# dRaniwal/RAJNI-ViT

Measured on AMD Instinct MI355X. Metric: images/sec ViT-B/16@224 with README schedule, higher is better.
Workload: dtype bf16

## Files before the change

include/rajni_hip_debug.h:

```cpp
#ifndef RAJNI_HIP_DEBUG_H
#define RAJNI_HIP_DEBUG_H

#include "rajni_hip.h"

#ifdef __cplusplus
extern "C" {
#endif

void rajni_debug_force_attention(int mode);

int rajni_debug_attention_rows(const void* qkv, const int32_t* keep_idx, void* out, int B, int n_src, int np, int nq,
                               int H, int D, float scale, int dtype, rajni_stream_t stream);

void rajni_debug_set_last_block_all_rows(int on);
int rajni_debug_last_block_cls_rows(const rajni_vit_plan* plan, const rajni_vit_ext* ext, const rajni_vit_prefix* prefix);

void rajni_debug_force_gemm_tiling(int mode);

void rajni_debug_force_f8_tiling(int mode);

void rajni_debug_set_resid_stagger(int units);

void rajni_debug_set_gemm_nblock_bytes(int bytes);

enum { RAJNI_TILING_SMALL = 1,
       RAJNI_TILING_F32 = 2,
       RAJNI_TILING_WIDE = 4,
       RAJNI_TILING_MID = 5,
       RAJNI_TILING_F8_STREAM = 8,
       RAJNI_TILING_F8_WIDE = 9 };
typedef struct rajni_linear_plan {
  int tiling;
  int tiles_n, total_tiles, nblk;
  int grid;
  int lds_bytes;
} rajni_linear_plan;
int rajni_debug_linear_plan(const rajni_linear_args* args, int cus, rajni_linear_plan* out);

void rajni_debug_force_score_two_pass(int on);

void rajni_debug_force_score_tiled(int on);

void rajni_debug_set_gemm_stamps(void* buf);

#ifdef __cplusplus
}
#endif
#endif
```

rajni-vit_amd/csrc/common.h:

```cpp
#pragma once
#include <hip/hip_runtime.h>
#include <stdint.h>
#include <stdio.h>
#include "../../include/rajni_hip.h"
#include "../../include/rajni_hip_debug.h"

typedef unsigned short bf16_t;
typedef __attribute__((ext_vector_type(8))) __bf16 bf16x8;
typedef __attribute__((ext_vector_type(2))) __bf16 bf16x2;
typedef __attribute__((ext_vector_type(4))) float f32x4;
typedef __attribute__((ext_vector_type(16))) float f32x16;
typedef __attribute__((ext_vector_type(4))) short s16x4;

#define LDS_PTR(p) ((__attribute__((address_space(3))) void*)(p))
#define GLB_PTR(p) ((const __attribute__((address_space(1))) void*)(p))

__device__ __forceinline__ float bf2f(bf16_t u) { return __uint_as_float(((unsigned)u) << 16); }
__device__ __forceinline__ bf16_t f2bf(float f) {
  __bf16 b = (__bf16)f;
  return __builtin_bit_cast(bf16_t, b);
}
__device__ __forceinline__ unsigned pack2bf(float lo, float hi) {
  bf16x2 v = {(__bf16)lo, (__bf16)hi};
  return __builtin_bit_cast(unsigned, v);
// ... 116 lines not shown
  KC_GEMM_BIAS = 0, KC_GEMM_GELU = 1, KC_GEMM_RESID = 2, KC_GEMM_PATCH = 3, KC_ATTENTION = 4,
  KC_LAYERNORM = 5, KC_SCORE_SELECT = 6, KC_IMPORTANCE = 7, KC_SELECT = 8, KC_GATHER = 9,
  KC_CLS_POS = 10, KC_OTHER = 11,
  KC_GEMM_RESID_SQ = 12,
  KC_GEMM8_BIAS = 13, KC_GEMM8_GELU = 14, KC_GEMM8_RESID = 15,
  KC_GEMM8_RESID_SQ = 16
};
struct ProfScope {
  int kc; hipStream_t s; void* rec;
  ProfScope(int kclass, hipStream_t stream, double flops, double bytes);
  ~ProfScope();
};

#define RAJNI_CHECK_LAUNCH(name)                                              \
  do {                                                                        \
    hipError_t e__ = hipGetLastError();                                       \
    if (e__ != hipSuccess) {                                                  \
      rajni_set_error("%s launch failed: %s", name, hipGetErrorString(e__));  \
      return RAJNI_ERR_LAUNCH;                                                \
    }                                                                         \
  } while (0)

#define RAJNI_REQUIRE(cond, code, ...)       \
  do {                                       \
    if (!(cond)) {                           \
      rajni_set_error(__VA_ARGS__);          \
      return code;                           \
    }                                        \
  } while (0)

extern unsigned long long* rajni_g_stamps;

int launch_linear(const rajni_linear_args& a, hipStream_t s);
int launch_patch_embed(const void* images, const void* w, const float* bias, const void* cls,
                       const void* pos, int pos_has_cls, void* x, int out_f32, int B, int Cin, int S,
                       int P, int C, int dtype, void* ws, size_t ws_bytes, hipStream_t s,
                       int num_prefix = 1, const void* reg = nullptr);
size_t patch_embed_workspace_bytes(int B, int Cin, int S, int P, int dtype);
int launch_layernorm(const void* x, long xs, const float* w, const float* b, void* y, int rows,
                     int C, float eps, int x_f32, int dtype, hipStream_t s);
int launch_layernorm_fp8(const void* x, long xs, const float* w, const float* b, void* yq, float* yscale,
                         float* hscale, float wnorm, float bmax, int rows, int C, float eps, int x_f32, hipStream_t s);
int launch_attention(const void* qkv, const int32_t* keep_idx, void* out, int B, int n_src, int np, int nq,
                     int H, int D, float scale, int dtype, hipStream_t s);
int launch_attention_fp8(const void* qkv, const int32_t* keep_idx, void* out_q, float out_scale, float* row_scale,
                         int B, int n_src, int np, int H, int D, float scale, hipStream_t s);
int launch_attention_cls(const void* qkv, void* out, int B, int N, int H, int D, float scale, int dtype,
                         hipStream_t s, float q_scale = 0.f);
int launch_score_select(const void* qkv, const void* scores_in, int B, int N, int H, int D,
                        float eps, int keep, void* scores_out, int32_t* keep_idx,
                        void* next_scores, int dtype, hipStream_t s, int num_prefix = 1, void* ws = nullptr,
                        size_t ws_bytes = 0);
int launch_gather_rows(const void* src, const int32_t* idx, void* dst, int B, int n_src, int n_dst,
                       int row_bytes, hipStream_t s);
int launch_qk_norm(void* qkv, const float* qw, const float* qb, const float* kw, const float* kb, int rows, int H, int D,
                   float eps, int dtype, hipStream_t s);
int launch_layernorm_stream(void* x, const float* w, const float* b, int rows, int C, float eps, int x_f32, int dtype, hipStream_t s);
int launch_pool_norm(const void* x, int B, int N, int C, int pool, const float* nw, const float* nb, float neps,
                     const float* fw, const float* fb, float feps, void* out, int x_f32, int dtype, hipStream_t s,
                     int num_prefix = 1);
```

rajni-vit_amd/csrc/forward.hip:

```cpp
#include "common.h"

namespace {

inline size_t align256(size_t v) { return (v + 255) & ~(size_t)255; }

struct Workspace {
  char *xa, *xb, *xn, *qkv, *att, *hid, *clsn, *scf, *cols;
  char* sst; size_t sst_bytes;
  float *xs, *hs;
  size_t total, cols_bytes;
};

Workspace carve(const rajni_vit_plan& p, int P) {
  const size_t gw = p.img_size / p.patch_size, n0 = gw * gw + P;
  const size_t rows = (size_t)p.B * n0, es = p.dtype == RAJNI_F32 ? 4 : 2, xs = (p.dtype == RAJNI_F32 || !p.resid_bf16) ? 4 : 2;
  Workspace w{};
  size_t off = 0;
  auto take = [&](size_t bytes) { size_t o = off; off += align256(bytes); return o; };
  const size_t oxa = take(rows * p.C * xs), oxb = take(rows * p.C * xs), oxn = take(rows * p.C * es);
  const size_t oqkv = take(rows * 3 * p.C * es), oatt = take(rows * p.C * es);
  const size_t ohid = take(rows * p.hidden * es), ocls = take((size_t)p.B * p.C * es);
  const size_t oscf = take(rows * es);
  w.cols_bytes = patch_embed_workspace_bytes(p.B, p.in_chans, p.img_size, p.patch_size, p.dtype);
  const size_t ocols = take(w.cols_bytes);
// ... 99 lines not shown
}
rajni_linear_args fc1_args(const Fwd& f, const rajni_block& blk, int M) {
  rajni_linear_args g = linear_args(f.p.dtype, f.w.xn, blk.fc1_w, blk.fc1_b, blk.fc1_s, f.w.hid, M, f.p.hidden, f.p.C, RAJNI_EPI_BIAS_GELU);
  if (f.p.act_fp8) { g.x_scale = f.w.xs; g.y_scale = f.w.hs; }
  return g;
}
rajni_linear_args fc2_args(const Fwd& f, const rajni_block& blk, int M, void* y) {
  rajni_linear_args g = linear_args(f.p.dtype, f.w.hid, blk.fc2_w, blk.fc2_b, blk.fc2_s, y, M, f.p.C, f.p.hidden, RAJNI_EPI_BIAS_RESID);
  if (f.p.act_fp8) g.x_scale = f.w.hs;
  g.gamma = blk.ls2; g.resid = y; g.ldr = f.p.C; g.stream_f32 = f.sf32;
  return g;
}

int layernorm(const Fwd& f, const void* x, const float* g, const float* b, int rows, float* hs = nullptr, float wnorm = 0.f,
              float bmax = 0.f) {
  const rajni_vit_plan& p = f.p;
  if (p.act_fp8) return launch_layernorm_fp8(x, p.C, g, b, f.w.xn, f.w.xs, hs, wnorm, bmax, rows, p.C, p.ln_eps, f.sf32, f.s);
  return launch_layernorm(x, p.C, g, b, f.w.xn, rows, p.C, p.ln_eps, f.sf32, p.dtype, f.s);
}

inline bool attn_emits_e4m3(const rajni_vit_plan& p, const rajni_block& blk, int np) {
  return p.act_fp8 && blk.attn_out_scale > 0.f && blk.proj_s != nullptr && p.D == 64 && np <= 224;
}

struct Tail { rajni_linear_args proj, fc1, fc2; };
Tail tail_args(const Fwd& f, const rajni_block& blk, const AttnRows& r, const void* x, void* y) {
  return Tail{proj_args(f, blk, r, x, y), fc1_args(f, blk, r.M), fc2_args(f, blk, r.M, y)};
}
bool tail_ok(const Tail& t) {
  rajni_linear_plan unused;
  return rajni_debug_linear_plan(&t.proj, 256, &unused) == RAJNI_OK && rajni_debug_linear_plan(&t.fc1, 256, &unused) == RAJNI_OK &&
         rajni_debug_linear_plan(&t.fc2, 256, &unused) == RAJNI_OK;
}
int launch_tail(const Fwd& f, const rajni_block& blk, const Tail& t) {
  int rc = launch_linear(t.proj, f.s);
  if (rc != RAJNI_OK) return rc;
  rc = layernorm(f, t.proj.y, blk.norm2_w, blk.norm2_b, t.proj.M, f.w.hs, blk.fc1_rownorm_max, blk.fc1_bias_absmax);
  if (rc != RAJNI_OK) return rc;
  rc = launch_linear(t.fc1, f.s);
  if (rc != RAJNI_OK) return rc;
  return launch_linear(t.fc2, f.s);
}

inline int prefix_count(const rajni_vit_prefix* pre) { return (pre && pre->num_prefix > 1) ? pre->num_prefix : 1; }

int check_prefix(const rajni_vit_prefix* pre, const char* who) {
  if (!pre) return RAJNI_OK;
  RAJNI_REQUIRE(pre->num_prefix >= 0 && pre->num_prefix <= RAJNI_MAX_PREFIX, RAJNI_ERR_INVALID,
                "%s: num_prefix must be 0..%d (%d)", who, RAJNI_MAX_PREFIX, pre->num_prefix);
  RAJNI_REQUIRE(pre->num_prefix <= 1 || pre->reg_token != nullptr, RAJNI_ERR_INVALID,
                "%s: %d prefix tokens but reg_token is null", who, pre->num_prefix);
  RAJNI_REQUIRE(pre->num_prefix > 1 || pre->reg_token == nullptr, RAJNI_ERR_INVALID,
                "%s: reg_token given but num_prefix is %d", who, pre->num_prefix);
  return RAJNI_OK;
}

inline int tokens_after(const rajni_block& blk, int N, int P) { return blk.keep > 0 ? blk.keep + P : N; }
int tokens_entering(const rajni_vit_plan& p, int P, int i) {
  const int gw = p.img_size / p.patch_size;
  int N = gw * gw + P;
  for (int j = 0; j < i; ++j) N = tokens_after(p.blocks[j], N, P);
  return N;
}

inline int logits_stride(const rajni_vit_plan& p) { return p.logits_ld > 0 ? p.logits_ld : p.num_classes; }

int check_schedule(const rajni_vit_plan& p, int P) {
  for (int i = 0; i < p.depth; ++i) {
    const rajni_block& blk = p.blocks[i];
    if (blk.keep <= 0) continue;
    const int patches = tokens_entering(p, P, i) - P;
    RAJNI_REQUIRE(blk.keep <= patches, RAJNI_ERR_INVALID, "block %d: keep=%d but only %d patch tokens", i, blk.keep, patches);
    RAJNI_REQUIRE(blk.keep_idx && blk.next_scores, RAJNI_ERR_INVALID, "block %d: keep_idx/next_scores buffers missing", i);
  }
// ... 66 lines not shown
  const Fwd f{p, w, (dt != RAJNI_F32 && !p.resid_bf16) ? 1 : 0, s};
  int N = tokens_entering(p, P, 0);

  rc = launch_patch_embed(images, p.patch_w, p.patch_b, p.cls_token, p.pos_embed, p.pos_has_cls,
                          w.xa, f.sf32, B, p.in_chans, p.img_size, p.patch_size, C, dt, w.cols, w.cols_bytes, s,
                          P, P > 1 ? pre->reg_token : nullptr);
  if (rc != RAJNI_OK) return rc;
  if (ext && ext->norm_pre_w) {
    rc = launch_layernorm_stream(w.xa, ext->norm_pre_w, ext->norm_pre_b, B * N, C, ext->norm_pre_eps, f.sf32, dt, s);
    if (rc != RAJNI_OK) return rc;
  }

  char* cur = w.xa;
  char* oth = w.xb;
  const void* carried = nullptr;

  for (int i = 0; i < p.depth; ++i) {
    const rajni_block& blk = p.blocks[i];
    if (p.token_counts) p.token_counts[i] = N;
    const int M = B * N;
    rc = layernorm(f, cur, blk.norm1_w, blk.norm1_b, M);
    if (rc != RAJNI_OK) return rc;
    rc = launch_linear(qkv_args(f, blk, M), s);
    if (rc != RAJNI_OK) return rc;
    if (qkn) {
      rc = launch_qk_norm(w.qkv, qkn[i].q_norm_w, qkn[i].q_norm_b, qkn[i].k_norm_w, qkn[i].k_norm_b, M, p.H, p.D, ext->qk_eps, dt, s);
      if (rc != RAJNI_OK) return rc;
    }

    const long cls_ld = (long)N * C;
    if (p.cls_only_last_block && i == p.depth - 1 && blk.keep == 0 && N > 1) {
      rc = launch_attention_cls(w.qkv, w.att, B, N, p.H, p.D, p.attn_scale, dt, s, attn_emits_e4m3(p, blk, N) ? blk.attn_out_scale : 0.f);
      if (rc != RAJNI_OK) return rc;
      rc = launch_tail(f, blk, tail_args(f, blk, AttnRows{B, C, nullptr, cls_ld, nullptr, 0, 0}, cur, oth));
      if (rc != RAJNI_OK) return rc;
      cur = oth; N = 1;
      break;
    }
    if (last_block_cls_rows(p, ext, i, N)) {
      const Tail t = tail_args(f, blk, AttnRows{B, cls_ld, nullptr, cls_ld, nullptr, 0, 0}, cur, oth);
      if (tail_ok(t)) {
        rc = launch_attention(w.qkv, nullptr, w.att, B, N, N, 1, p.H, p.D, p.attn_scale, dt, s);
        if (rc != RAJNI_OK) return rc;
        rc = launch_tail(f, blk, t);
        if (rc != RAJNI_OK) return rc;
        cur = oth; N = 1;
        break;
      }
    }

    const int Np = tokens_after(blk, N, P);
    const int32_t* idx = nullptr;
    if (blk.keep > 0) {
      const bool recompute = blk.update || carried == nullptr;
      if (blk.forced_keep_idx) {
        const void* full = carried;
        if (recompute) {
          void* dst = blk.scores ? blk.scores : (void*)w.scf;
          rc = launch_score_select(w.qkv, nullptr, B, N, p.H, p.D, 1e-6f, 0, dst, nullptr, nullptr, dt, s, 1, w.sst, w.sst_bytes);
          if (rc != RAJNI_OK) return rc;
          full = dst;
        }
        const int n = B * Np;
        if (dt == RAJNI_F32)
          hipLaunchKernelGGL(carry_scores_kernel<float>, dim3((n + 255) / 256), dim3(256), 0, s,
                             (const float*)full, blk.forced_keep_idx, (float*)blk.next_scores, B, N, Np);
        else
          hipLaunchKernelGGL(carry_scores_kernel<bf16_t>, dim3((n + 255) / 256), dim3(256), 0, s,
                             (const bf16_t*)full, blk.forced_keep_idx, (bf16_t*)blk.next_scores, B, N, Np);
        RAJNI_CHECK_LAUNCH("carry_scores_kernel");
        idx = blk.forced_keep_idx;
      } else {
        if (recompute)
          rc = launch_score_select(w.qkv, nullptr, B, N, p.H, p.D, 1e-6f, blk.keep, blk.scores,
                                   blk.keep_idx, blk.next_scores, dt, s, P, w.sst, w.sst_bytes);
        else
          rc = launch_score_select(nullptr, carried, B, N, 0, 0, 0.f, blk.keep, nullptr,
                                   blk.keep_idx, blk.next_scores, dt, s, P);
        if (rc != RAJNI_OK) return rc;
        idx = blk.keep_idx;
      }
      carried = blk.next_scores;
    } else {
      carried = nullptr;
    }

    const bool att8 = attn_emits_e4m3(p, blk, Np);
    if (att8) rc = launch_attention_fp8(w.qkv, idx, w.att, blk.attn_out_scale, w.xs, B, N, Np, p.H, p.D, p.attn_scale, s);
    else rc = launch_attention(w.qkv, idx, w.att, B, N, Np, Np, p.H, p.D, p.attn_scale, dt, s);
    if (rc != RAJNI_OK) return rc;
    char* y = idx ? oth : cur;
    rc = launch_tail(f, blk, tail_args(f, blk, AttnRows{B * Np, C, att8 ? w.xs : nullptr, C, idx, Np, N}, cur, y));
    if (rc != RAJNI_OK) return rc;
    if (idx) { oth = cur; cur = y; }
    N = Np;
  }

  if (ext && (ext->pool != RAJNI_POOL_TOKEN || ext->fc_norm_w || ext->norm_absent))
    rc = launch_pool_norm(cur, B, N, C, ext->pool, ext->norm_absent ? nullptr : p.norm_w, p.norm_b, p.ln_eps,
                          ext->fc_norm_w, ext->fc_norm_b, ext->fc_norm_eps, w.clsn, f.sf32, dt, s, P);
  else
    rc = launch_layernorm(cur, (long)N * C, p.norm_w, p.norm_b, w.clsn, B, C, p.ln_eps, f.sf32, dt, s);
  if (rc != RAJNI_OK) return rc;
  rajni_linear_args head = linear_args(dt, w.clsn, p.head_w, p.head_b, nullptr, logits, B, p.num_classes, C, RAJNI_EPI_BIAS);
  head.ldc = logits_stride(p);
  return launch_linear(head, s);
}

}
```

rajni-vit_amd/csrc/gemm.hip:

```cpp
#include <stdlib.h>
#include <type_traits>
#include "common.h"

namespace {

enum { EPI_BIAS = 0, EPI_GELU = 1, EPI_RESID = 2, EPI_PATCH = 3,
       EPI_GELU8 = 4 };
enum { ALOAD_PLAIN = 0, ALOAD_PATCH = 1 };

struct GemmParams {
  const void* X; long lda;
  const void* W; long ldw;
  const float* wscale;
  const float* xscale;
  const float* yscale;
  const float* bias;
  const float* gamma;
  const void* R; long ldr;
  const int* ridx; int r_np, r_nsrc;
  void* Y; long ldc;
  int M, N, K;
  int tiles_n, total_tiles;
  int nblk;
  int cin, S, log2ps, gw, npatch;
// ... 903 lines not shown
  pre.valid = false;
  stage(0, 0);
  for (int kt = 0; kt < nk; ++kt) {
    asm volatile("s_waitcnt vmcnt(0)" ::: "memory");
    __syncthreads();
    if (kt + 1 < nk) stage(kt + 1, (kt + 1) & 1);
    else prefetch_resid<EPI, SF32, 4>(p, pre, m0 + wm * 64, n0 + wn * 64, l15, g);
    const char* sx = smem + (kt & 1) * STAGE_BYTES;
    const char* sw = sx + TILE_BYTES;
#pragma unroll
    for (int ks = 0; ks < 2; ++ks) {
      const int c = ks * 4 + g;
      bf16x8 xf[4], wf[4];
#pragma unroll
      for (int i = 0; i < 4; ++i) {
        xf[i] = *reinterpret_cast<const bf16x8*>(sx + xoff[i] + ((c ^ xkey[i]) << 4));
        if constexpr (W8)
          wf[i] = w_frag_bf16(*reinterpret_cast<const WFrag*>(sw + woff[i] + (((c >> 1) ^ wkey[i]) << 4) + ((c & 1) << 3)));
        else
          wf[i] = *reinterpret_cast<const bf16x8*>(sw + woff[i] + ((c ^ wkey[i]) << 4));
      }
#pragma unroll
      for (int ni = 0; ni < 4; ++ni)
#pragma unroll
        for (int mi = 0; mi < 4; ++mi)
          acc[ni][mi] = mfma_16x16x32<A>(wf[ni], xf[mi], acc[ni][mi]);
    }
  }

  epilogue_tile<A, EPI, SF32, 4, W8>(p, acc, m0 + wm * 64, n0 + wn * 64, l15, g, pre);
}
}

#include "gemm_f8.h"

namespace f32 {
constexpr int BM = 128, BN = 128, BK = 32;
constexpr int TILE_BYTES = BM * BK * 4;
constexpr int STAGE_BYTES = 2 * TILE_BYTES;
constexpr int LDS_BYTES = 2 * STAGE_BYTES;
using small::key_w;
using small::key_x;

template <int EPI>
__device__ __forceinline__ void epilogue_row_f32(const GemmParams& p, int m, int nb, float* v, const float* gam) {
  long orow = m;
  if (EPI == EPI_GELU) {
#pragma unroll
    for (int j = 0; j < 16; ++j) v[j] = 0.5f * v[j] * (1.0f + erff(v[j] * 0.70710678118654752f));
  } else if (EPI == EPI_RESID) {
    long rrow = m;
    if (p.ridx != nullptr) {
      const int b = m / p.r_np;
      rrow = (long)b * p.r_nsrc + p.ridx[m];
    }
    const long roff = rrow * p.ldr + nb;
#pragma unroll
    for (int j = 0; j < 16; ++j)
      if (nb + j < p.N) v[j] = fmaf(gam[j], v[j], reinterpret_cast<const float*>(p.R)[roff + j]);
  } else if (EPI == EPI_PATCH) {
    const int b = m / p.npatch, pp = m - b * p.npatch;
    orow = (long)b * (p.npatch + p.nprefix) + p.nprefix + pp;
    const float* pr = reinterpret_cast<const float*>(p.pos) + (long)(pp + p.pos_off) * p.ldc + nb;
#pragma unroll
    for (int j = 0; j < 16; ++j)
      if (nb + j < p.N) v[j] += pr[j];
// ... 194 lines not shown
  if ((mode == 4 || mode == 5) && p.M < 256) mode = 1;
  if (mode == 4 && p.K < 192) mode = 1;
  if (mode == 5 && p.K < 256) mode = 1;
  const long resid_rows = p.ridx != nullptr ? (long)(p.M / p.r_np) * p.r_nsrc : (long)p.M;
  const bool mid_ok = !r.resid_nat || resid_rows * p.ldr < (1L << 31);
  if (mode == 5 && !mid_ok) mode = 1;
  if (mode == 0) {
    if (p.M >= 1024 && p.N >= 1536 && p.K >= 192) mode = 4;
    else if (p.M >= 1024 && p.K >= 256) mode = (p.K > p.N && p.K >= 1536 && wide_wins_on_rounds(p.M, p.N, cus)) ? 4 : (mid_ok ? 5 : 1);
    else mode = 1;
  }
  if (mode == 4) return make_plan(p, RAJNI_TILING_WIDE, 256, 256, r.lds_wide, cus, 2, nblk_bytes);
  if (mode == 5) return make_plan(p, RAJNI_TILING_MID, 256, 128, r.lds_narrow, cus, 2, nblk_bytes);
  return make_plan(p, RAJNI_TILING_SMALL, 128, 128, small::LDS_BYTES);
}

rajni_linear_plan choose_gemm_f8(const GemmParams& p, const TileTraits& r, int cus, int force, int nblk_bytes) {
  if (r.lds_wide != 0) {
    const bool wide_ok = p.K >= 384;
    auto rounds_ok = [&]() {
      const double rounds = (double)((p.M + 255) / 256) * ((p.N + f8w::BN - 1) / f8w::BN) / cus;
      const double frac = rounds - (long)rounds;
      return !(rounds < 8.0 && frac > 0.0 && frac < 0.2);
    };
    const bool want = force == 2 ||
                      (force == 0 && p.M >= 1024 && p.N >= 1536 && (r.epi == EPI_GELU8 || (RAJNI_F8W_LINES && rounds_ok())));
    if (wide_ok && want) return make_plan(p, RAJNI_TILING_F8_WIDE, 256, f8w::BN, r.lds_wide, cus, 1, nblk_bytes);
  }
  return make_plan(p, RAJNI_TILING_F8_STREAM, 256, f8::BN, r.lds_narrow, cus, 1, nblk_bytes);
}

int g_resid_stagger = 1;

struct LaunchCtl { int kclass; bool sq; hipStream_t s; int cus; rajni_linear_plan* plan_only; };
inline int cus_of(const LaunchCtl& l) { return l.cus > 0 ? l.cus : rajni_num_cus(); }

template <auto Kernel>
int launch_planned(const rajni_linear_plan& c, int threads, GemmParams& p, const LaunchCtl& l, double bytes, const char* name) {
  if (l.plan_only != nullptr) { *l.plan_only = c; return RAJNI_OK; }
  static bool done_by_device[RAJNI_MAX_DEVICES] = {};
  bool& done = done_by_device[rajni_current_device()];
  if (!done) {
    hipError_t e = hipFuncSetAttribute(reinterpret_cast<const void*>(Kernel), hipFuncAttributeMaxDynamicSharedMemorySize, c.lds_bytes);
    if (e != hipSuccess) {
      rajni_set_error("hipFuncSetAttribute(gemm): %s", hipGetErrorString(e));
      return RAJNI_ERR_LAUNCH;
    }
    done = true;
  }
  p.tiles_n = c.tiles_n; p.total_tiles = c.total_tiles; p.nblk = c.nblk;
  ProfScope prof(l.kclass, l.s, 2.0 * p.M * (double)p.N * p.K, bytes);
  hipLaunchKernelGGL(Kernel, dim3(c.grid), dim3(threads), c.lds_bytes, l.s, p);
  RAJNI_CHECK_LAUNCH(name);
  return RAJNI_OK;
}
inline double gemm_bytes(const GemmParams& p, double xsz, double wsz, double ysz) {
  return xsz * (double)p.M * p.K + ysz * (double)p.M * p.N + wsz * (double)p.N * p.K;
}
constexpr double out_bytes(int epi, bool sf32) {
  const double ysz = epi == EPI_GELU8 ? 1.0 : (sf32 && (epi == EPI_RESID || epi == EPI_PATCH)) ? 4.0 : 2.0;
  return ysz + (epi == EPI_RESID ? (sf32 ? 4.0 : 2.0) : 0.0);
}

template <int EPI, int ALOAD, bool SF32, bool W8, typename A, int WM, int WN, int MI, int NS>
int launch_stream(const rajni_linear_plan& c, GemmParams& p, const LaunchCtl& l, double bytes) {
  if constexpr (EPI == EPI_RESID)
    if (l.sq) return launch_planned<&wide::gemm_bf16_tn_stream<EPI, ALOAD, SF32, WM, WN, MI, NS, W8, 1, A>>(c, 512, p, l, bytes, "gemm_bf16_tn");
// ... 7 lines not shown
  p.stamps = rajni_g_stamps;
  p.stagger = g_resid_stagger;
  const double bytes = gemm_bytes(p, 2.0, W8 ? 1.0 : 2.0, out_bytes(EPI, SF32));
  if (c.tiling == RAJNI_TILING_WIDE) return launch_stream<EPI, ALOAD, SF32, W8, A, 2, 4, 8, NS>(c, p, l, bytes);
  if (c.tiling == RAJNI_TILING_MID) return launch_stream<EPI, ALOAD, SF32, W8, A, 4, 2, 4, 3>(c, p, l, bytes);
  return launch_planned<&small::gemm_bf16_tn_128x128<EPI, ALOAD, SF32, W8, A>>(c, 256, p, l, bytes, "gemm_bf16_tn");
}
template <int EPI, bool SF32>
int launch_gemm_f8(GemmParams& p, const LaunchCtl& l) {
  constexpr bool HAS_WIDE = EPI == EPI_BIAS || EPI == EPI_GELU8;
  constexpr TileTraits T{EPI, resid_nat(EPI, SF32), HAS_WIDE ? f8w::lds_bytes(EPI) : 0, f8::lds_bytes(EPI, SF32)};
  const rajni_linear_plan c = choose_gemm_f8(p, T, cus_of(l), g_force_f8_tiling, g_nblk_bytes);
  p.stamps = rajni_g_stamps;
  const double bytes = gemm_bytes(p, 1.0, 1.0, out_bytes(EPI, SF32));
  if constexpr (HAS_WIDE)
    if (c.tiling == RAJNI_TILING_F8_WIDE) return launch_planned<&f8w::gemm_f8_tn_wide<EPI>>(c, 512, p, l, bytes, "gemm_f8_tn_wide");
  if constexpr (EPI == EPI_RESID)
    if (l.sq) return launch_planned<&f8::gemm_f8_tn_stream<EPI, SF32, 1>>(c, 512, p, l, bytes, "gemm_f8_tn");
  return launch_planned<&f8::gemm_f8_tn_stream<EPI, SF32, 0>>(c, 512, p, l, bytes, "gemm_f8_tn");
}
template <int EPI, int ALOAD>
int launch_gemm_f32(GemmParams& p, const LaunchCtl& l) {
  return launch_planned<&f32::gemm_f32_tn_128x128<EPI, ALOAD>>(make_plan(p, RAJNI_TILING_F32, 128, 128, f32::LDS_BYTES), 256, p, l,
                                                              gemm_bytes(p, 4.0, 4.0, 4.0), "gemm_f32_tn");
}

enum { FMT_F8F8, FMT_W8, FMT_F32, FMT_BF16, FMT_F16 };
template <bool W8, typename A>
int linear16(int epi, bool sf32, GemmParams& p, const LaunchCtl& l) {
  return epi == EPI_BIAS ? launch_gemm<EPI_BIAS, ALOAD_PLAIN, false, W8, A>(p, l)
       : epi == EPI_GELU ? launch_gemm<EPI_GELU, ALOAD_PLAIN, false, W8, A>(p, l)
       : sf32 ? launch_gemm<EPI_RESID, ALOAD_PLAIN, true, W8, A>(p, l) : launch_gemm<EPI_RESID, ALOAD_PLAIN, false, W8, A>(p, l);
}
int linear(const rajni_linear_args& a, LaunchCtl l) {
  RAJNI_REQUIRE(a.dtype == RAJNI_BF16 || a.dtype == RAJNI_F32 || a.dtype == RAJNI_F16, RAJNI_ERR_INVALID,
                "rajni_linear: bad dtype %d", a.dtype);
  RAJNI_REQUIRE(a.dtype != RAJNI_F16 || (a.w_scale == nullptr && a.x_scale == nullptr), RAJNI_ERR_UNSUPPORTED,
                "rajni_linear: fp8 weights or activations need a bf16 model (dtype fp16 given)");
  RAJNI_REQUIRE(a.x && a.w && a.y, RAJNI_ERR_INVALID, "rajni_linear: null pointer");
  RAJNI_REQUIRE(a.M > 0 && a.N > 0 && a.K > 0 && a.K % 64 == 0, RAJNI_ERR_INVALID,
                "rajni_linear: M,N>0 and K %% 64 == 0 required (M=%d N=%d K=%d)", a.M, a.N, a.K);
  RAJNI_REQUIRE(a.lda % 8 == 0 && a.ldw % 8 == 0 && a.ldc % 8 == 0, RAJNI_ERR_INVALID,
                "rajni_linear: leading dimensions must be multiples of 8 elements");
  RAJNI_REQUIRE(((uintptr_t)a.x | (uintptr_t)a.w | (uintptr_t)a.y | (uintptr_t)a.resid) % 16 == 0,
                RAJNI_ERR_INVALID, "rajni_linear: pointers must be 16-byte aligned");
  GemmParams p{};
  p.X = a.x; p.lda = a.lda;
  p.W = a.w; p.ldw = a.ldw;
  p.bias = a.bias; p.gamma = a.gamma;
  p.R = a.resid; p.ldr = a.ldr;
  p.ridx = a.r_idx; p.r_np = a.r_np > 0 ? a.r_np : 1; p.r_nsrc = a.r_nsrc;
  p.Y = a.y; p.ldc = a.ldc;
  p.M = a.M; p.N = a.N; p.K = a.K;
  p.wscale = a.w_scale;
  const int fmt = a.x_scale != nullptr ? FMT_F8F8 : a.w_scale != nullptr ? FMT_W8
                : a.dtype == RAJNI_F32 ? FMT_F32 : a.dtype == RAJNI_F16 ? FMT_F16 : FMT_BF16;
  const bool f8 = fmt == FMT_F8F8;
  if (f8) {
    RAJNI_REQUIRE(a.w_scale != nullptr && a.dtype == RAJNI_BF16, RAJNI_ERR_INVALID,
                  "rajni_linear: fp8 activations (x_scale) need fp8 weights (w_scale) and dtype bf16");
    RAJNI_REQUIRE(a.K % 256 == 0 && a.K >= 512, RAJNI_ERR_UNSUPPORTED,
                  "rajni_linear: the fp8 x fp8 kernel needs K %% 256 == 0 and K >= 512 (K=%d)", a.K);
    RAJNI_REQUIRE(a.lda % 16 == 0 && a.ldw % 16 == 0, RAJNI_ERR_INVALID, "rajni_linear: fp8 operands need lda, ldw %% 16 == 0 (bytes)");
    p.xscale = a.x_scale; p.yscale = a.y_scale;
  } else {
    RAJNI_REQUIRE(a.y_scale == nullptr, RAJNI_ERR_INVALID, "rajni_linear: y_scale without x_scale");
    if (fmt == FMT_W8) {
      RAJNI_REQUIRE(a.dtype == RAJNI_BF16, RAJNI_ERR_UNSUPPORTED, "rajni_linear: fp8 weights need bf16 activations");
      RAJNI_REQUIRE(a.ldw % 16 == 0, RAJNI_ERR_INVALID, "rajni_linear: fp8 weights need ldw %% 16 == 0");
    }
  }
  int epi;
  switch (a.epilogue) {
    case RAJNI_EPI_BIAS:
      RAJNI_REQUIRE(!f8 || a.y_scale == nullptr, RAJNI_ERR_UNSUPPORTED, "rajni_linear: an fp8 output (y_scale) exists for the GELU epilogue only");
      epi = EPI_BIAS; l.kclass = f8 ? KC_GEMM8_BIAS : KC_GEMM_BIAS;
      break;
    case RAJNI_EPI_BIAS_GELU:
      RAJNI_REQUIRE(!f8 || (a.y_scale != nullptr && a.ldc % 16 == 0), RAJNI_ERR_UNSUPPORTED,
                    "rajni_linear: the fp8 x fp8 GELU epilogue writes e4m3 (y_scale required, ldc %% 16 == 0 bytes)");
      epi = f8 ? EPI_GELU8 : EPI_GELU; l.kclass = f8 ? KC_GEMM8_GELU : KC_GEMM_GELU;
      break;
    case RAJNI_EPI_BIAS_RESID:
      if (f8) RAJNI_REQUIRE(a.resid != nullptr && a.ldr % 8 == 0 && a.y_scale == nullptr, RAJNI_ERR_INVALID,
                            "rajni_linear: RESID epilogue needs resid, ldr %% 8 == 0 and no y_scale");
      else if (fmt == FMT_F32) RAJNI_REQUIRE(a.resid != nullptr, RAJNI_ERR_INVALID, "rajni_linear: RESID epilogue needs resid");
      else RAJNI_REQUIRE(a.resid != nullptr && a.ldr % 8 == 0, RAJNI_ERR_INVALID,
                         "rajni_linear: RESID epilogue needs resid and ldr %% 8 == 0");
      epi = EPI_RESID; l.sq = a.K <= a.N;
      l.kclass = f8 ? (l.sq ? KC_GEMM8_RESID_SQ : KC_GEMM8_RESID) : (l.sq ? KC_GEMM_RESID_SQ : KC_GEMM_RESID);
      break;
    default:
      rajni_set_error("rajni_linear: unknown epilogue %d", a.epilogue);
      return RAJNI_ERR_INVALID;
  }
  const bool sf32 = a.stream_f32 != 0;
  switch (fmt) {
    case FMT_F8F8: return epi == EPI_BIAS ? launch_gemm_f8<EPI_BIAS, false>(p, l) : epi == EPI_GELU8 ? launch_gemm_f8<EPI_GELU8, false>(p, l)
                        : sf32 ? launch_gemm_f8<EPI_RESID, true>(p, l) : launch_gemm_f8<EPI_RESID, false>(p, l);
    case FMT_F32: return epi == EPI_BIAS ? launch_gemm_f32<EPI_BIAS, ALOAD_PLAIN>(p, l) : epi == EPI_GELU ? launch_gemm_f32<EPI_GELU, ALOAD_PLAIN>(p, l)
                       : launch_gemm_f32<EPI_RESID, ALOAD_PLAIN>(p, l);
    case FMT_W8: return linear16<true, bf16_t>(epi, sf32, p, l);
    case FMT_F16: return linear16<false, f16_t>(epi, sf32, p, l);
    default: return linear16<false, bf16_t>(epi, sf32, p, l);
  }
}

}

extern "C" void rajni_debug_force_gemm_tiling(int mode) { g_force_tiling = mode; }
extern "C" void rajni_debug_force_f8_tiling(int mode) { g_force_f8_tiling = mode; }
extern "C" void rajni_debug_set_resid_stagger(int units) { g_resid_stagger = units; }
extern "C" void rajni_debug_set_gemm_nblock_bytes(int bytes) { g_nblk_bytes = bytes; }
extern "C" void rajni_debug_set_gemm_stamps(void* buf) { rajni_g_stamps = (unsigned long long*)buf; }

int launch_linear(const rajni_linear_args& a, hipStream_t s) { return linear(a, LaunchCtl{0, false, s, 0, nullptr}); }
extern "C" int rajni_debug_linear_plan(const rajni_linear_args* args, int cus, rajni_linear_plan* out) {
  RAJNI_REQUIRE(args != nullptr, RAJNI_ERR_INVALID, "rajni_linear: null args");
  RAJNI_REQUIRE(out != nullptr && cus > 0, RAJNI_ERR_INVALID, "rajni_debug_linear_plan: needs out and cus > 0");
  return linear(*args, LaunchCtl{0, false, nullptr, cus, out});
}

static bool patch_fused(int Cin, int S, int P) {
  return P >= 8 && (P & (P - 1)) == 0 && S % 8 == 0 && (Cin * P * P) % 64 == 0;
}
size_t patch_embed_workspace_bytes(int B, int Cin, int S, int P, int dtype) {
  if (P <= 0 || S <= 0 || S % P != 0 || patch_fused(Cin, S, P)) return 0;
  const size_t kpad = ((size_t)Cin * P * P + 63) / 64 * 64, gw = S / P;
  return (size_t)B * gw * gw * kpad * (dtype == RAJNI_F32 ? 4 : 2);
}
template <typename T>
__global__ void __launch_bounds__(256) im2col_kernel(const T* img, T* cols, int Cin, int S, int P, int gw, int kpad, long total8) {
  const long i = (long)blockIdx.x * blockDim.x + threadIdx.x;
  if (i >= total8) return;
  const int k8 = kpad >> 3;
  const long m = i / k8;
  const int k0 = (int)(i - m * k8) * 8;
  const int npatch = gw * gw;
  const int b = (int)(m / npatch), pp = (int)(m - (long)b * npatch);
  const int gy = pp / gw, gx = pp - gy * gw;
  const int K = Cin * P * P;
  T v[8];
#pragma unroll
  for (int j = 0; j < 8; ++j) {
    const int k = k0 + j;
    T e = T(0);
    if (k < K) {
      const int c = k / (P * P), r = k - c * P * P, py = r / P, px = r - py * P;
      e = img[(((long)b * Cin + c) * S + gy * P + py) * S + gx * P + px];
// ... 92 lines not shown
```

rajni-vit_amd/rajni_amd/_native.py:

```python
from __future__ import annotations

import ctypes as C
import os
from typing import Optional

import torch

_HERE = os.path.dirname(os.path.abspath(__file__))
LIB_PATH = os.environ.get("RAJNI_HIP_LIB") or os.path.join(_HERE, "lib", "librajni_hip.so")

RAJNI_F32, RAJNI_BF16, RAJNI_F16 = 0, 1, 2
EPI_BIAS, EPI_BIAS_GELU, EPI_BIAS_RESID = 0, 1, 2
NUM_KCLASS = 17
POOL_TOKEN, POOL_AVG = 0, 1

c_void_p, c_int, c_long, c_float, c_size_t = C.c_void_p, C.c_int, C.c_long, C.c_float, C.c_size_t


class NativeError(RuntimeError):
    pass


class LinearArgs(C.Structure):
    _fields_ = [("x", c_void_p), ("lda", c_long), ("w", c_void_p), ("ldw", c_long),
# ... 55 lines not shown


MAX_PREFIX = 32
SCORE_TILE_TOKENS = 32
SCORE_TILED_MAX_TOKENS = 16384 + MAX_PREFIX

_SIGS = {
    "rajni_abi_version": (c_int, []),
    "rajni_last_error": (C.c_char_p, []),
    "rajni_device_check": (c_int, []),
    "rajni_importance": (c_int, [c_void_p, c_void_p, c_int, c_int, c_int, c_int, c_float, c_int, c_void_p]),
    "rajni_select_topk": (c_int, [c_void_p, c_int, c_int, c_int, c_void_p, c_void_p, c_int, c_void_p]),
    "rajni_score_select": (c_int, [c_void_p, c_int, c_int, c_int, c_int, c_float, c_int, c_void_p, c_void_p,
                                   c_void_p, c_int, c_void_p]),
    "rajni_gather_rows": (c_int, [c_void_p, c_void_p, c_void_p, c_int, c_int, c_int, c_int, c_int, c_void_p]),
    "rajni_attention": (c_int, [c_void_p, c_void_p, c_void_p, c_int, c_int, c_int, c_int, c_int, c_float,
                                c_int, c_void_p]),
    "rajni_attention_fp8": (c_int, [c_void_p, c_void_p, c_void_p, c_float, c_void_p, c_int, c_int, c_int, c_int, c_int, c_float,
                                    c_void_p]),
    "rajni_layernorm": (c_int, [c_void_p, c_long, c_void_p, c_void_p, c_void_p, c_int, c_int, c_float,
                                c_int, c_int, c_void_p]),
    "rajni_layernorm_fp8": (c_int, [c_void_p, c_long, c_void_p, c_void_p, c_void_p, c_void_p, c_void_p, c_float, c_float,
                                    c_int, c_int, c_float, c_int, c_void_p]),
    "rajni_linear": (c_int, [C.POINTER(LinearArgs), c_void_p]),
    "rajni_qk_norm": (c_int, [c_void_p, c_void_p, c_void_p, c_void_p, c_void_p, c_int, c_int, c_int, c_float, c_int, c_void_p]),
    "rajni_layernorm_stream": (c_int, [c_void_p, c_void_p, c_void_p, c_int, c_int, c_float, c_int, c_int, c_void_p]),
    "rajni_pool_norm": (c_int, [c_void_p, c_int, c_int, c_int, c_int, c_void_p, c_void_p, c_float, c_void_p, c_void_p, c_float,
                                c_void_p, c_int, c_int, c_void_p]),
    "rajni_debug_force_gemm_tiling": (None, [c_int]),
    "rajni_debug_force_f8_tiling": (None, [c_int]),
    "rajni_debug_set_resid_stagger": (None, [c_int]),
    "rajni_debug_set_gemm_nblock_bytes": (None, [c_int]),
    "rajni_debug_linear_plan": (c_int, [C.POINTER(LinearArgs), c_int, C.POINTER(LinearPlan)]),
    "rajni_debug_force_attention": (None, [c_int]),
    "rajni_debug_attention_rows": (c_int, [c_void_p, c_void_p, c_void_p, c_int, c_int, c_int, c_int, c_int, c_int, c_float,
                                           c_int, c_void_p]),
    "rajni_debug_set_last_block_all_rows": (None, [c_int]),
    "rajni_debug_last_block_cls_rows": (c_int, [C.POINTER(VitPlan), C.POINTER(VitExt), C.POINTER(VitPrefix)]),
    "rajni_debug_force_score_two_pass": (None, [c_int]),
    "rajni_debug_force_score_tiled": (None, [c_int]),
    "rajni_debug_set_gemm_stamps": (None, [c_void_p]),
    "rajni_patch_embed_workspace_bytes": (c_size_t, [c_int, c_int, c_int, c_int, c_int]),
    "rajni_patch_embed": (c_int, [c_void_p, c_void_p, c_void_p, c_void_p, c_void_p, c_int, c_void_p, c_int, c_int,
                                  c_int, c_int, c_int, c_int, c_int, c_void_p, c_size_t, c_void_p]),
    "rajni_vit_workspace_bytes": (c_size_t, [C.POINTER(VitPlan)]),
    "rajni_vit_forward": (c_int, [C.POINTER(VitPlan), c_void_p, c_void_p, c_void_p]),
    "rajni_vit_forward_ext": (c_int, [C.POINTER(VitPlan), C.POINTER(VitExt), c_void_p, c_void_p, c_void_p]),
    "rajni_select_topk_prefix": (c_int, [c_void_p, c_int, c_int, c_int, c_int, c_void_p, c_void_p, c_int, c_void_p]),
    "rajni_score_select_prefix": (c_int, [c_void_p, c_int, c_int, c_int, c_int, c_float, c_int, c_int, c_void_p, c_void_p,
                                          c_void_p, c_int, c_void_p]),
    "rajni_score_select_workspace_bytes": (c_size_t, [c_int, c_int, c_int, c_int, c_int]),
    "rajni_score_select_ws": (c_int, [c_void_p, c_int, c_int, c_int, c_int, c_float, c_int, c_int, c_void_p, c_void_p,
                                      c_void_p, c_int, c_void_p, c_size_t, c_void_p]),
    "rajni_patch_embed_prefix": (c_int, [c_void_p, c_void_p, c_void_p, c_void_p, c_void_p, c_int, c_void_p, c_int, c_void_p,
                                         c_int, c_int, c_int, c_int, c_int, c_int, c_int, c_void_p, c_size_t, c_void_p]),
    "rajni_pool_norm_prefix": (c_int, [c_void_p, c_int, c_int, c_int, c_int, c_int, c_void_p, c_void_p, c_float, c_void_p,
                                       c_void_p, c_float, c_void_p, c_int, c_int, c_void_p]),
    "rajni_vit_workspace_bytes_prefix": (c_size_t, [C.POINTER(VitPlan), C.POINTER(VitPrefix)]),
    "rajni_vit_forward_ext_prefix": (c_int, [C.POINTER(VitPlan), C.POINTER(VitExt), C.POINTER(VitPrefix), c_void_p, c_void_p,
                                             c_void_p]),
    "rajni_profile_enable": (None, [C.c_uint]),
    "rajni_profile_class_name": (C.c_char_p, [c_int]),
    "rajni_profile_collect": (c_int, [C.POINTER(C.c_longlong), C.POINTER(C.c_double), C.POINTER(C.c_double),
                                      C.POINTER(C.c_double)]),
    "rajni_profile_reset": (None, []),
}
# ... 104 lines not shown
```

Baseline: 30040.

## Add few-row bf16 GEMM kernel for CLS-only last block and head

Adds a dedicated bf16/f16 GEMM kernel with 16-row-per-wave tiles and a deep global-to-LDS ring for small-M linears. It is used for the proj/fc1/fc2 of the CLS-only last block and for the classifier head. The goal is to avoid wasting a large M tile and to spread the work across more CUs when M equals the batch size. The catch is that it skips any fp8 path in those layers, because it is only eligible when there are no scales. It also adds more kernel variants.

```diff
diff --git a/include/rajni_hip_debug.h b/include/rajni_hip_debug.h
--- a/include/rajni_hip_debug.h
+++ b/include/rajni_hip_debug.h
@@ -37,6 +37,10 @@
 } rajni_linear_plan;
 int rajni_debug_linear_plan(const rajni_linear_args* args, int cus, rajni_linear_plan* out);
 
+int rajni_debug_linear_rows(const rajni_linear_args* args, rajni_stream_t stream);
+int rajni_debug_linear_rows_eligible(const rajni_linear_args* args);
+void rajni_debug_set_linear_rows_waves(int waves);
+
 void rajni_debug_force_score_two_pass(int on);
 
 void rajni_debug_force_score_tiled(int on);
diff --git a/rajni-vit_amd/csrc/common.h b/rajni-vit_amd/csrc/common.h
--- a/rajni-vit_amd/csrc/common.h
+++ b/rajni-vit_amd/csrc/common.h
@@ -172,6 +172,7 @@
 extern unsigned long long* rajni_g_stamps;
 
 int launch_linear(const rajni_linear_args& a, hipStream_t s);
+int launch_linear_rows(const rajni_linear_args& a, hipStream_t s);
 int launch_patch_embed(const void* images, const void* w, const float* bias, const void* cls,
                        const void* pos, int pos_has_cls, void* x, int out_f32, int B, int Cin, int S,
                        int P, int C, int dtype, void* ws, size_t ws_bytes, hipStream_t s,
diff --git a/rajni-vit_amd/csrc/forward.hip b/rajni-vit_amd/csrc/forward.hip
--- a/rajni-vit_amd/csrc/forward.hip
+++ b/rajni-vit_amd/csrc/forward.hip
@@ -155,14 +155,15 @@
   return rajni_debug_linear_plan(&t.proj, 256, &unused) == RAJNI_OK && rajni_debug_linear_plan(&t.fc1, 256, &unused) == RAJNI_OK &&
          rajni_debug_linear_plan(&t.fc2, 256, &unused) == RAJNI_OK;
 }
-int launch_tail(const Fwd& f, const rajni_block& blk, const Tail& t) {
-  int rc = launch_linear(t.proj, f.s);
+int launch_tail(const Fwd& f, const rajni_block& blk, const Tail& t, bool few_rows = false) {
+  const auto linear = few_rows ? launch_linear_rows : launch_linear;
+  int rc = linear(t.proj, f.s);
   if (rc != RAJNI_OK) return rc;
   rc = layernorm(f, t.proj.y, blk.norm2_w, blk.norm2_b, t.proj.M, f.w.hs, blk.fc1_rownorm_max, blk.fc1_bias_absmax);
   if (rc != RAJNI_OK) return rc;
-  rc = launch_linear(t.fc1, f.s);
-  if (rc != RAJNI_OK) return rc;
-  return launch_linear(t.fc2, f.s);
+  rc = linear(t.fc1, f.s);
+  if (rc != RAJNI_OK) return rc;
+  return linear(t.fc2, f.s);
 }
 
 inline int prefix_count(const rajni_vit_prefix* pre) { return (pre && pre->num_prefix > 1) ? pre->num_prefix : 1; }
@@ -295,7 +296,7 @@
     if (p.cls_only_last_block && i == p.depth - 1 && blk.keep == 0 && N > 1) {
       rc = launch_attention_cls(w.qkv, w.att, B, N, p.H, p.D, p.attn_scale, dt, s, attn_emits_e4m3(p, blk, N) ? blk.attn_out_scale : 0.f);
       if (rc != RAJNI_OK) return rc;
-      rc = launch_tail(f, blk, tail_args(f, blk, AttnRows{B, C, nullptr, cls_ld, nullptr, 0, 0}, cur, oth));
+      rc = launch_tail(f, blk, tail_args(f, blk, AttnRows{B, C, nullptr, cls_ld, nullptr, 0, 0}, cur, oth), true);
       if (rc != RAJNI_OK) return rc;
       cur = oth; N = 1;
       break;
@@ -305,7 +306,7 @@
       if (tail_ok(t)) {
         rc = launch_attention(w.qkv, nullptr, w.att, B, N, N, 1, p.H, p.D, p.attn_scale, dt, s);
         if (rc != RAJNI_OK) return rc;
-        rc = launch_tail(f, blk, t);
+        rc = launch_tail(f, blk, t, true);
         if (rc != RAJNI_OK) return rc;
         cur = oth; N = 1;
         break;
@@ -367,7 +368,7 @@
   if (rc != RAJNI_OK) return rc;
   rajni_linear_args head = linear_args(dt, w.clsn, p.head_w, p.head_b, nullptr, logits, B, p.num_classes, C, RAJNI_EPI_BIAS);
   head.ldc = logits_stride(p);
-  return launch_linear(head, s);
-}
-
-}
+  return launch_linear_rows(head, s);
+}
+
+}
diff --git a/rajni-vit_amd/csrc/gemm.hip b/rajni-vit_amd/csrc/gemm.hip
--- a/rajni-vit_amd/csrc/gemm.hip
+++ b/rajni-vit_amd/csrc/gemm.hip
@@ -959,6 +959,127 @@
 }
 }
 
+namespace rows {
+constexpr int BN = 64, BK = 64;
+constexpr int W_BYTES = BN * BK * 2;
+constexpr int XW_BYTES = 16 * BK * 2;
+template <int WM> struct Cfg {
+  static constexpr int BM = 16 * WM;
+  static constexpr int STAGE_BYTES = W_BYTES + WM * XW_BYTES;
+  static constexpr int PW = 8 / WM;
+  static constexpr int PIECES = 2 + PW;
+  static constexpr int NS = 63 / PIECES + 1 < 8 ? 63 / PIECES + 1 : 8;
+  static constexpr int LDS_BYTES = NS * STAGE_BYTES;
+};
+template <int PIECES, int NS>
+__device__ __forceinline__ void wait_steps_left(int steps) {
+  static_assert(NS <= 8, "one case per step of the ring");
+  switch (steps) {
+    case 0: wide::wait_step<0>(); break;
+    case 1: wide::wait_step<(NS > 2 ? 1 : 0) * PIECES>(); break;
+    case 2: wide::wait_step<(NS > 3 ? 2 : 0) * PIECES>(); break;
+    case 3: wide::wait_step<(NS > 4 ? 3 : 0) * PIECES>(); break;
+    case 4: wide::wait_step<(NS > 5 ? 4 : 0) * PIECES>(); break;
+    case 5: wide::wait_step<(NS > 6 ? 5 : 0) * PIECES>(); break;
+    default: wide::wait_step<(NS > 7 ? 6 : 0) * PIECES>(); break;
+  }
+}
+
+template <int EPI, bool SF32, typename A, int WM>
+__global__ void __launch_bounds__(WM * 64) gemm_bf16_tn_rows(const GemmParams p) {
+  using C = Cfg<WM>;
+  constexpr int MAP = col_map(EPI, SF32);
+  constexpr int NS = C::NS, PW = C::PW;
+  extern __shared__ __attribute__((aligned(16))) char smem[];
+  const int tid = threadIdx.x, lane = tid & 63;
+  const int wave = __builtin_amdgcn_readfirstlane(tid >> 6);
+  const int t = xcd_tile(p.total_tiles);
+  const int tiles_m = p.total_tiles / p.tiles_n;
+  const int tn = t / tiles_m, tm = t - tn * tiles_m;
+  const int m0 = tm * C::BM + wave * 16, n0 = tn * BN;
+
+  const int r_in = lane >> 3, pch = lane & 7;
+  const char* xs[2];
+  const char* ws[PW];
+#pragma unroll
+  for (int i = 0; i < 2; ++i) {
+    const int row = i * 8 + r_in;
+    int m = m0 + row;
+    if (m > p.M - 1) m = p.M - 1;
+    xs[i] = reinterpret_cast<const char*>(p.X) + ((long)m * p.lda + (pch ^ small::key_x(row)) * 8) * 2;
+  }
+#pragma unroll
+  for (int i = 0; i < PW; ++i) {
+    const int row = (wave * PW + i) * 8 + r_in;
+    int n = n0 + row;
+    if (n > p.N - 1) n = p.N - 1;
+    ws[i] = reinterpret_cast<const char*>(p.W) + ((long)n * p.ldw + (pch ^ w_key<MAP>(row)) * 8) * 2;
+  }
+  auto stage = [&](int kt, int buf) {
+    char* sw = smem + buf * C::STAGE_BYTES;
+    char* sx = sw + W_BYTES + wave * XW_BYTES;
+    const int k0 = kt * BK;
+#pragma unroll
+    for (int i = 0; i < PW; ++i)
+      __builtin_amdgcn_global_load_lds(GLB_PTR(ws[i] + k0 * 2), LDS_PTR(sw + (wave * PW + i) * 1024), 16, 0, 0);
+#pragma unroll
+    for (int i = 0; i < 2; ++i)
+      __builtin_amdgcn_global_load_lds(GLB_PTR(xs[i] + k0 * 2), LDS_PTR(sx + i * 1024), 16, 0, 0);
+  };
+
+  const int l15 = lane & 15, g = lane >> 4;
+  const int xoff = l15 * 128, xkey = small::key_x(l15);
+  int woff[4], wkey[4];
+#pragma unroll
+  for (int i = 0; i < 4; ++i) {
+    const int wr = w_frag_row<MAP>(l15, i);
+    woff[i] = wr * 128; wkey[i] = w_key<MAP>(wr);
+  }
+  f32x4 acc[4][1];
+#pragma unroll
+  for (int a = 0; a < 4; ++a) acc[a][0] = f32x4{0.f, 0.f, 0.f, 0.f};
+  auto compute = [&](int buf) {
+    const char* sw = smem + buf * C::STAGE_BYTES;
+    const char* sx = sw + W_BYTES + wave * XW_BYTES;
+#pragma unroll
+    for (int ks = 0; ks < 2; ++ks) {
+      const int c = ks * 4 + g;
+      bf16x8 wf[4];
+      const bf16x8 xf = *reinterpret_cast<const bf16x8*>(sx + xoff + ((c ^ xkey) << 4));
+#pragma unroll
+      for (int i = 0; i < 4; ++i) wf[i] = *reinterpret_cast<const bf16x8*>(sw + woff[i] + ((c ^ wkey[i]) << 4));
+#pragma unroll
+      for (int ni = 0; ni < 4; ++ni) acc[ni][0] = mfma_16x16x32<A>(wf[ni], xf, acc[ni][0]);
+    }
+  };
+
+  const int nk = p.K / BK;
+  const int ahead = nk < NS - 1 ? nk : NS - 1;
+  for (int j = 0; j < ahead; ++j) stage(j, j);
+  int buf = 0;
+  for (int kt = 0; kt < nk - ahead; ++kt) {
+    wide::wait_step<(NS - 2) * C::PIECES>();
+    __builtin_amdgcn_s_barrier();
+    asm volatile("" ::: "memory");
+    stage(kt + NS - 1, buf == 0 ? NS - 1 : buf - 1);
+    compute(buf);
+    buf = buf + 1 == NS ? 0 : buf + 1;
+  }
+  ResidPrefetch<1> pre;
+  pre.valid = false;
+  for (int left = ahead - 1; left >= 0; --left) {
+    wait_steps_left<C::PIECES, NS>(left);
+    __builtin_amdgcn_s_barrier();
+    asm volatile("" ::: "memory");
+    if (left == 0) prefetch_resid<EPI, SF32, 1>(p, pre, m0, n0, l15, g);
+    compute(buf);
+    buf = buf + 1 == NS ? 0 : buf + 1;
+  }
+  const bool interior = m0 + 16 <= p.M && n0 + BN <= p.N;
+  epilogue_tile<A, EPI, SF32, 1, false>(p, acc, m0, n0, l15, g, pre, 0, interior);
+}
+}
+
 #include "gemm_f8.h"
 
 namespace f32 {
@@ -1219,7 +1340,8 @@
 
 int g_resid_stagger = 1;
 
-struct LaunchCtl { int kclass; bool sq; hipStream_t s; int cus; rajni_linear_plan* plan_only; };
+struct LaunchCtl { int kclass; bool sq; hipStream_t s; int cus; rajni_linear_plan* plan_only;
+                   bool rows; };
 inline int cus_of(const LaunchCtl& l) { return l.cus > 0 ? l.cus : rajni_num_cus(); }
 
 template <auto Kernel>
@@ -1293,6 +1415,37 @@
        : epi == EPI_GELU ? launch_gemm<EPI_GELU, ALOAD_PLAIN, false, W8, A>(p, l)
        : sf32 ? launch_gemm<EPI_RESID, ALOAD_PLAIN, true, W8, A>(p, l) : launch_gemm<EPI_RESID, ALOAD_PLAIN, false, W8, A>(p, l);
 }
+
+int g_rows_wm = 0;
+constexpr int ROWS_WM = 4;
+constexpr int ROWS_MAX_M = 512;
+inline bool rows_eligible(const rajni_linear_args& a) {
+  return (a.dtype == RAJNI_BF16 || a.dtype == RAJNI_F16) && a.w_scale == nullptr && a.x_scale == nullptr && a.y_scale == nullptr &&
+         a.r_idx == nullptr && a.M > 0 && a.M <= ROWS_MAX_M && a.N > 0 && a.K > 0 && a.K % 64 == 0 &&
+         (a.epilogue == RAJNI_EPI_BIAS || a.epilogue == RAJNI_EPI_BIAS_GELU || a.epilogue == RAJNI_EPI_BIAS_RESID);
+}
+template <int EPI, bool SF32, typename A, int WM>
+int launch_rows_wm(GemmParams& p, const LaunchCtl& l) {
+  using C = rows::Cfg<WM>;
+  rajni_linear_plan c{};
+  c.tiles_n = (p.N + rows::BN - 1) / rows::BN;
+  c.grid = c.total_tiles = c.tiles_n * ((p.M + C::BM - 1) / C::BM);
+  c.lds_bytes = C::LDS_BYTES;
+  return launch_planned<&rows::gemm_bf16_tn_rows<EPI, SF32, A, WM>>(c, WM * 64, p, l, gemm_bytes(p, 2.0, 2.0, out_bytes(EPI, SF32)),
+                                                                   "gemm_bf16_tn_rows");
+}
+template <int EPI, bool SF32, typename A>
+int launch_rows(GemmParams& p, const LaunchCtl& l) {
+  const int wm = g_rows_wm > 0 ? g_rows_wm : ROWS_WM;
+  return wm == 1 ? launch_rows_wm<EPI, SF32, A, 1>(p, l) : wm == 2 ? launch_rows_wm<EPI, SF32, A, 2>(p, l)
+                                                                   : launch_rows_wm<EPI, SF32, A, 4>(p, l);
+}
+template <typename A>
+int linear_rows16(int epi, bool sf32, GemmParams& p, const LaunchCtl& l) {
+  return epi == EPI_BIAS ? launch_rows<EPI_BIAS, false, A>(p, l) : epi == EPI_GELU ? launch_rows<EPI_GELU, false, A>(p, l)
+       : sf32 ? launch_rows<EPI_RESID, true, A>(p, l) : launch_rows<EPI_RESID, false, A>(p, l);
+}
+
 int linear(const rajni_linear_args& a, LaunchCtl l) {
   RAJNI_REQUIRE(a.dtype == RAJNI_BF16 || a.dtype == RAJNI_F32 || a.dtype == RAJNI_F16, RAJNI_ERR_INVALID,
                 "rajni_linear: bad dtype %d", a.dtype);
@@ -1356,6 +1509,7 @@
       return RAJNI_ERR_INVALID;
   }
   const bool sf32 = a.stream_f32 != 0;
+  if (l.rows && rows_eligible(a)) return fmt == FMT_F16 ? linear_rows16<f16_t>(epi, sf32, p, l) : linear_rows16<bf16_t>(epi, sf32, p, l);
   switch (fmt) {
     case FMT_F8F8: return epi == EPI_BIAS ? launch_gemm_f8<EPI_BIAS, false>(p, l) : epi == EPI_GELU8 ? launch_gemm_f8<EPI_GELU8, false>(p, l)
                         : sf32 ? launch_gemm_f8<EPI_RESID, true>(p, l) : launch_gemm_f8<EPI_RESID, false>(p, l);
@@ -1375,7 +1529,15 @@
 extern "C" void rajni_debug_set_gemm_nblock_bytes(int bytes) { g_nblk_bytes = bytes; }
 extern "C" void rajni_debug_set_gemm_stamps(void* buf) { rajni_g_stamps = (unsigned long long*)buf; }
 
+extern "C" void rajni_debug_set_linear_rows_waves(int waves) { g_rows_wm = (waves == 1 || waves == 2 || waves == 4) ? waves : 0; }
+
 int launch_linear(const rajni_linear_args& a, hipStream_t s) { return linear(a, LaunchCtl{0, false, s, 0, nullptr}); }
+int launch_linear_rows(const rajni_linear_args& a, hipStream_t s) { return linear(a, LaunchCtl{0, false, s, 0, nullptr, true}); }
+extern "C" int rajni_debug_linear_rows(const rajni_linear_args* args, rajni_stream_t stream) {
+  RAJNI_REQUIRE(args != nullptr, RAJNI_ERR_INVALID, "rajni_linear: null args");
+  return launch_linear_rows(*args, (hipStream_t)stream);
+}
+extern "C" int rajni_debug_linear_rows_eligible(const rajni_linear_args* args) { return args != nullptr && rows_eligible(*args) ? 1 : 0; }
 extern "C" int rajni_debug_linear_plan(const rajni_linear_args* args, int cus, rajni_linear_plan* out) {
   RAJNI_REQUIRE(args != nullptr, RAJNI_ERR_INVALID, "rajni_linear: null args");
   RAJNI_REQUIRE(out != nullptr && cus > 0, RAJNI_ERR_INVALID, "rajni_debug_linear_plan: needs out and cus > 0");
diff --git a/rajni-vit_amd/rajni_amd/_native.py b/rajni-vit_amd/rajni_amd/_native.py
--- a/rajni-vit_amd/rajni_amd/_native.py
+++ b/rajni-vit_amd/rajni_amd/_native.py
@@ -111,6 +111,9 @@
     "rajni_debug_set_resid_stagger": (None, [c_int]),
     "rajni_debug_set_gemm_nblock_bytes": (None, [c_int]),
     "rajni_debug_linear_plan": (c_int, [C.POINTER(LinearArgs), c_int, C.POINTER(LinearPlan)]),
+    "rajni_debug_linear_rows": (c_int, [C.POINTER(LinearArgs), c_void_p]),
+    "rajni_debug_linear_rows_eligible": (c_int, [C.POINTER(LinearArgs)]),
+    "rajni_debug_set_linear_rows_waves": (None, [c_int]),
     "rajni_debug_force_attention": (None, [c_int]),
     "rajni_debug_attention_rows": (c_int, [c_void_p, c_void_p, c_void_p, c_int, c_int, c_int, c_int, c_int, c_int, c_float,
                                            c_int, c_void_p]),
```

Result: no change. 30330 (median of 6 runs) (+0.9%).
